# amazon-science/gan-control

Measured on AMD Instinct MI355X. Metric: images/sec G+D step FFHQ-1024, higher is better.
Workload: dtype bf16x3; 1 GPU; FFHQ 1024x1024 full G+D train step (D step, G step, lazy R1 every 16 and path-length every 4, Adam, EMA), 4 images/GPU, fp32 storage, conv arithmetic bf16x3; global_batch=4, parallelism=dp1

## Files before the change

### gan-control_amd/csrc/bias_act.hip

```cpp
#include "common.h"

namespace {

__device__ __forceinline__ float lrelu_gain(float v, float slope, float gain) {
    return (v > 0.f ? v : v * slope) * gain;
}

template <bool VEC, bool NOISE>
__global__ __launch_bounds__(256) void bias_act_plane_kernel(
    const float* __restrict__ x, const float* __restrict__ bias, const float* __restrict__ noise,
    const float* __restrict__ noise_w, float* __restrict__ y, int channels, int64_t inner, float slope, float gain) {
    const int plane = blockIdx.y;
    const int c = plane % channels, b = plane / channels;
    const float bv = bias ? bias[c] : 0.f;
    const float nw = NOISE ? noise_w[0] : 0.f;
    const float* xp = x + (size_t)plane * inner;
    float* yp = y + (size_t)plane * inner;
    const float* np = NOISE ? noise + (size_t)b * inner : nullptr;
    if (VEC) {
        const int64_t n4 = inner >> 2;
        for (int64_t i = (int64_t)blockIdx.x * 256 + threadIdx.x; i < n4; i += (int64_t)gridDim.x * 256) {
            const gc::f32x4_t xv = gc::stream_load4(xp + 4 * i);
            float4 v = make_float4(xv.x, xv.y, xv.z, xv.w);
            if (NOISE) {
// ... 487 lines not shown
    int chunks, rpc;
    plane_dot_pitched_plan(rows, &chunks, &rpc);
    return chunks;
}

extern "C" int gc_plane_dot_pitched_f32(const float* a, const float* b, float* partial, int planes, int rows, int width, int a_pitch, int b_pitch,
                                        gc_stream_t stream) {
    if (!a || !b || !partial) return gc::fail(GC_ERR_BAD_ARG, "gc_plane_dot_pitched_f32: null pointer");
    if (planes <= 0 || rows <= 0 || width <= 0 || a_pitch < width || b_pitch < width) return gc::fail(GC_ERR_BAD_ARG, "gc_plane_dot_pitched_f32: bad extents");
    int chunks, rpc;
    plane_dot_pitched_plan(rows, &chunks, &rpc);
    if ((int64_t)planes * chunks > INT32_MAX) return gc::fail(GC_ERR_UNSUPPORTED, "gc_plane_dot_pitched_f32: more than 2^31 blocks");
    hipLaunchKernelGGL(plane_dot_pitched_kernel, dim3((unsigned)planes * (unsigned)chunks), dim3(256), 0, (hipStream_t)stream,
                       a, b, partial, rows, width, a_pitch, b_pitch, chunks, rpc);
    return gc::check_launch("gc_plane_dot_pitched_f32");
}

extern "C" int gc_rows_sum_div_f32(const float* partial, const float* den, float* out, int rows, int chunks, gc_stream_t stream) {
    if (!partial || !out) return gc::fail(GC_ERR_BAD_ARG, "gc_rows_sum_div_f32: null pointer");
    if (rows <= 0 || chunks <= 0) return gc::fail(GC_ERR_BAD_ARG, "gc_rows_sum_div_f32: bad extents");
    hipLaunchKernelGGL(rows_sum_div_kernel, dim3((unsigned)((rows + 255) / 256)), dim3(256), 0, (hipStream_t)stream, partial, den, out, rows, chunks);
    return gc::check_launch("gc_rows_sum_div_f32");
}

extern "C" int gc_plane_dot_f32(const float* a, const float* b, float* partial, int planes, int64_t inner, gc_stream_t stream) {
    if (!a || !b || !partial) return gc::fail(GC_ERR_BAD_ARG, "gc_plane_dot_f32: null pointer");
    if (planes <= 0 || inner <= 0) return gc::fail(GC_ERR_BAD_ARG, "gc_plane_dot_f32: bad extents");
    int chunks; int64_t len;
    channel_sum_plan(inner, &chunks, &len);
    if ((int64_t)planes * chunks > INT32_MAX) return gc::fail(GC_ERR_UNSUPPORTED, "gc_plane_dot_f32: more than 2^31 blocks");
    hipLaunchKernelGGL(plane_dot_kernel, dim3((unsigned)chunks * (unsigned)planes), dim3(256), 0, (hipStream_t)stream, a, b, partial, inner, chunks, len);
    return gc::check_launch("gc_plane_dot_f32");
}
```

### gan-control_amd/gan_control_amd/_lib.py

```python
import ctypes
import os

import torch

_HERE = os.path.dirname(os.path.abspath(__file__))
_DEFAULT = os.path.normpath(os.path.join(_HERE, '..', 'csrc', 'libgancontrol_hip.so'))

ABI_VERSION = 2
MODE_IDS = {'f32': 0, 'bf16x3': 1, 'bf16': 2}

_i32, _i64, _f32, _vp, _sz = ctypes.c_int32, ctypes.c_int64, ctypes.c_float, ctypes.c_void_p, ctypes.c_size_t


class ConvDesc(ctypes.Structure):
    _fields_ = [(n, _i32) for n in ('batch', 'in_ch', 'out_ch', 'in_h', 'in_w', 'out_h', 'out_w',
                                    'kh', 'kw', 'up', 'down', 'pad_y', 'pad_x', 'in_pitch', 'out_pitch')]


class ConvEpilogue(ctypes.Structure):
    _fields_ = [('bias', _vp), ('noise', _vp), ('noise_w', _vp), ('slope', _f32), ('gain', _f32), ('activate', _i32), ('residual', _vp)]


class GlinGroup(ctypes.Structure):
    _fields_ = [('x', _vp), ('w', _vp), ('bias', _vp), ('y', _vp), ('n', _i32), ('k', _i32), ('x_stride', _i64), ('alpha', _f32), ('beta', _f32)]


class WLayoutGroup(ctypes.Structure):
    _fields_ = [('src', _vp), ('dst', _vp), ('taps', _i32), ('k', _i32), ('n', _i32), ('flip_taps', _i32), ('src_stride', _i64 * 3), ('dst_stride', _i64 * 3), ('scale', _f32)]


class WPackGroup(ctypes.Structure):
    _fields_ = [('desc', ConvDesc), ('w', _vp), ('packed', _vp), ('packed_bytes', _sz)]


class WsqGroup(ctypes.Structure):
    _fields_ = [('w', _vp), ('g', _vp), ('out', _vp), ('rows', _i32), ('taps', _i32)]


STRUCTS = (ConvDesc, ConvEpilogue, WLayoutGroup, WPackGroup, GlinGroup, WsqGroup)

SIGNATURES = {
    'gc_abi_version': (_i32, []),
    'gc_last_error': (ctypes.c_char_p, []),
    'gc_struct_sizes': (_i32, [ctypes.POINTER(_sz), _i32]),
    'gc_source_hash': (ctypes.c_char_p, []),
    'gc_upfirdn2d_f32': (_i32, [_vp, _vp, _vp] + [_i32] * 14 + [_vp]),
    'gc_upfirdn2d_act_f32': (_i32, [_vp, _vp, _vp] + [_i32] * 11 + [_vp, _vp, _vp, _f32, _f32, _vp]),
    'gc_bias_act_f32': (_i32, [_vp, _vp, _vp, _vp, _vp, _i32, _i32, _i64, _f32, _f32, _vp]),
    'gc_bias_act_bwd_f32': (_i32, [_vp, _vp, _vp, _i64, _f32, _f32, _vp]),
    'gc_bias_act_bwd_noise_f32': (_i32, [_vp, _vp, _vp, _vp, _vp, _i32, _i32, _i64, _f32, _f32, _vp]),
    'gc_bias_act_bwd_chunks': (_i32, [_i64]),
    'gc_bias_act_bwd_reduce_f32': (_i32, [_vp, _vp, _vp, _vp, _vp, _vp, _i32, _i32, _i64, _f32, _f32, _vp]),
    'gc_bias_act_bwd_reduce_self_f32': (_i32, [_vp, _vp, _vp, _vp, _vp, _vp, _vp, _vp, _vp, _i32, _i32, _i64, _f32, _f32, _vp]),
    'gc_bias_act_bwd_reduce_adjoint_f32': (_i32, [_vp] * 13 + [_i32, _i32, _i64, _f32, _f32, _vp]),
    'gc_plane_dot_f32': (_i32, [_vp, _vp, _vp, _i32, _i64, _vp]),
    'gc_rows_sum_div_f32': (_i32, [_vp, _vp, _vp, _i32, _i32, _vp]),
    'gc_conv2d_bn_relu_f32': (_i32, [_vp, _vp, _vp, _vp, _vp] + [_i32] * 13 + [_vp]),
    'gc_pool2d_f32': (_i32, [_vp, _vp] + [_i32] * 10 + [_vp]),
    'gc_global_avgpool_f32': (_i32, [_vp, _vp, _i32, _i32, _vp]),
    'gc_resize_bilinear_f32': (_i32, [_vp, _vp, _i32, _i32, _i32, _i32, _i32, _f32, _f32, _vp]),
    'gc_channel_sum_workspace': (_sz, [_i32, _i32, _i64]),
    'gc_channel_sum_f32': (_i32, [_vp, _vp, _i32, _i32, _i64, _vp, _sz, _vp]),
    'gc_conv2d_f32': (_i32, [ctypes.POINTER(ConvDesc), _vp, _vp, _vp, _vp, _vp, _vp]),
    'gc_conv2d_fused_f32': (_i32, [ctypes.POINTER(ConvDesc), _vp, _vp, _vp, _vp, ctypes.POINTER(ConvEpilogue), _vp, _vp]),
    'gc_conv2d_f32_workspace': (_sz, [ctypes.POINTER(ConvDesc)]),
    'gc_small_gemm_ok': (_i32, [_i32, _i32, _i32, _i64, _i64]),
    'gc_small_gemm_f32': (_i32, [_vp, _i64, _i64, _vp, _i64, _i64, _vp, _f32, _f32, _vp, _i32, _i32, _i32, _vp]),
    'gc_conv2d_fused_f32_ws': (_i32, [ctypes.POINTER(ConvDesc), _vp, _vp, _vp, _vp, ctypes.POINTER(ConvEpilogue), _vp, _vp, _sz, _vp]),
    'gc_conv2d_fused_bf16x3_f32': (_i32, [ctypes.POINTER(ConvDesc), _vp, _vp, _vp, _vp, ctypes.POINTER(ConvEpilogue), _vp, _vp, _sz, _vp]),
    'gc_conv2d_bf16x3_workspace': (_sz, [ctypes.POINTER(ConvDesc)]),
    'gc_conv2d_bf16x3_packed_bytes': (_sz, [ctypes.POINTER(ConvDesc)]),
    'gc_conv2d_bf16x3_splitk_bytes': (_sz, [ctypes.POINTER(ConvDesc)]),
    'gc_conv2d_pack_weights_bf16x3': (_i32, [ctypes.POINTER(ConvDesc), _vp, _vp, _sz, _vp]),
    'gc_conv2d_fused_bf16x3_packed_f32': (_i32, [ctypes.POINTER(ConvDesc), _vp, _vp, _vp, _sz, _vp, _vp, ctypes.POINTER(ConvEpilogue), _vp, _vp, _sz, _vp]),
    'gc_conv2d_fused_bf16_packed_f32': (_i32, [ctypes.POINTER(ConvDesc), _vp, _vp, _vp, _sz, _vp, _vp, ctypes.POINTER(ConvEpilogue), _vp, _vp, _sz, _vp]),
    'gc_conv2d_wgrad_bf16_f32': (_i32, [ctypes.POINTER(ConvDesc), _vp, _vp, _vp, _vp, _vp, _vp, _sz, _vp]),
    'gc_conv2d_variant_name': (_i32, [ctypes.POINTER(ConvDesc), _i32, ctypes.c_char_p, _i32]),
    'gc_conv2d_wgrad_variant_name': (_i32, [ctypes.POINTER(ConvDesc), _i32, _i32, ctypes.c_char_p, _i32]),
    'gc_conv2d_out_pitch': (_i32, [ctypes.POINTER(ConvDesc), _i32]),
    'gc_conv2d_in_pitch_ok': (_i32, [ctypes.POINTER(ConvDesc), _i32, _i32]),
    'gc_upfirdn2d_variant_name': (_i32, [_i32] * 7 + [ctypes.c_char_p, _i32]),
    'gc_upfirdn2d_actbwd_tiles': (_i32, [_i32, _i32]),
    'gc_upfirdn2d_actbwd_f32': (_i32, [_vp] * 7 + [_i32] * 12 + [_f32, _f32, _vp]),
    'gc_upfirdn2d_mask_f32': (_i32, [_vp, _vp, _vp] + [_i32] * 12 + [_vp, _f32, _f32, _vp]),
    'gc_upfirdn2d_pitched_f32': (_i32, [_vp, _vp, _vp] + [_i32] * 14 + [_vp, _vp, _vp, _f32, _f32, _vp]),
    'gc_plane_dot_pitched_chunks': (_i32, [_i32]),
    'gc_plane_dot_pitched_f32': (_i32, [_vp, _vp, _vp, _i32, _i32, _i32, _i32, _i32, _vp]),
    'gc_conv2d_bf16x3_f32': (_i32, [ctypes.POINTER(ConvDesc), _vp, _vp, _vp, _vp, _vp, _vp, _sz, _vp]),
    'gc_conv2d_wgrad_workspace': (_sz, [ctypes.POINTER(ConvDesc)]),
# ... 142 lines not shown
```

### gan-control_amd/gan_control_amd/models/op/modulated_conv.py

```python
import math
import os

import torch
from torch.autograd import Function

from . import _backend
from ._backend import ConvGeom
from .conv2d_gradfix import _adjoint_geom, _adjoint_weight
from .weight_layout import kernel_layout
from .upfirdn2d import upfirdn2d, _dense_or_pitched


_WGRAD_SAMPLES = int(os.environ.get('GANCONTROL_WGRAD_SAMPLES', '1'))
_SAMPLES_MIN_RATIO = float(os.environ.get('GANCONTROL_WGRAD_SAMPLES_RATIO', '2'))


def _samples_route(x, gy, g, want_si, want_so, derived=False):
    if not _WGRAD_SAMPLES or torch.is_grad_enabled() or not (want_si or want_so) or (derived and _WGRAD_SAMPLES < 2):
        return False
    be = _backend.get()
    if not hasattr(be, 'conv2d_wgrad_samples_bytes'):
        return False
    saved = 2.0 * ((x.numel() if want_si else 0) + (gy.numel() if want_so else 0))
    extra = 3.0 * x.shape[0] * g.kh * g.kw * x.shape[1] * gy.shape[1]
    if saved < _SAMPLES_MIN_RATIO * extra:
        return False
    if g.up == 1:
        return be.conv2d_wgrad_samples_bytes(_dense_or_pitched(x), gy, g) > 0
    return be.conv2d_wgrad_samples_bytes(_dense_or_pitched(gy), x, _swapped_geom(g, x)) > 0


def _weight_and_scale_grads(x, gy, w_t, si, so, g, want_si, want_so):
    be = _backend.get()
    cs = lambda t: None if t is None else t.contiguous()
    if g.up == 1:
        gw, dws = be.conv2d_wgrad_samples(_dense_or_pitched(x), _dense_or_pitched(gy), cs(si), cs(so), g)
        gsi, gso = be.wgrad_samples_contract(dws, w_t.contiguous(), cs(si), cs(so), want_si, want_so)
        return gw, gsi, gso
    dw_adj, dws = be.conv2d_wgrad_samples(_dense_or_pitched(gy), _dense_or_pitched(x), cs(so), cs(si), _swapped_geom(g, x))
# ... 46 lines not shown
        ws = ctx.saved_tensors
        be = _backend.get()
        if torch.is_grad_enabled() or getattr(be, 'weight_sq_bwd', None) is None or not all(w.is_contiguous() for w in ws):
            return tuple((2.0 * g)[:, :, None, None] * w if ctx.needs_input_grad[i] else None for i, (g, w) in enumerate(zip(gs, ws)))
        idx = [i for i in range(len(ws)) if ctx.needs_input_grad[i]]
        outs = be.weight_sq_bwd([ws[i] for i in idx], [gs[i].contiguous() for i in idx]) if idx else []
        res = [None] * len(ws)
        for i, o in zip(idx, outs):
            res[i] = o
        return tuple(res)


def weight_sq_all(weights):
    return list(_backend.call(_WeightSqAll, *[w.view(w.shape[-4:]) for w in weights]))


def demod_coefficients(weight, s, scale, eps=1e-8):
    wsq = _backend.call(_WeightSq, weight.view(weight.shape[1:]))
    from .linear import equal_linear
    return torch.rsqrt(equal_linear(s.pow(2), wsq, _eps_vector(s, wsq.shape[0], eps), scale * scale, 1.0))


_EPS_VECTORS = {}


def _eps_vector(like, n, eps):
    key = (like.device, like.dtype, n, eps)
    t = _EPS_VECTORS.get(key)
    if t is None:
        t = _EPS_VECTORS[key] = torch.full((n,), eps, device=like.device, dtype=like.dtype)
    return t


class _SafeDiv(Function):

    @staticmethod
    def forward(ctx, num, den):
        out = _backend.get().rows_sum_div(num.contiguous().unsqueeze(-1), den.contiguous())
        ctx.save_for_backward(den, out)
        ctx.set_materialize_grads(False)
        return out

    @staticmethod
    def backward(ctx, g):
        if g is None:
            return None, None
        den, out = ctx.saved_tensors
        gq = _backend.call(_SafeDiv, g, den)
        return (gq if ctx.needs_input_grad[0] else None), (-(gq * out) if ctx.needs_input_grad[1] else None)


class _SumDiv(Function):

    @staticmethod
    def forward(ctx, partial, den):
        out = _backend.get().rows_sum_div(partial.contiguous(), den.contiguous())
        ctx.save_for_backward(den, out)
        ctx.chunks = partial.shape[-1]
        ctx.set_materialize_grads(False)
        return out

    @staticmethod
    def backward(ctx, g):
        if g is None:
            return None, None
        den, out = ctx.saved_tensors
        gq = _backend.call(_SafeDiv, g, den)
        return (gq.unsqueeze(-1).expand(*gq.shape, ctx.chunks) if ctx.needs_input_grad[0] else None), (-(gq * out) if ctx.needs_input_grad[1] else None)


class _PlaneDot(Function):

    @staticmethod
    def forward(ctx, a, b, den=None):
        out = _backend.get().plane_dot(_dense_or_pitched(a), _dense_or_pitched(b), den)
        ctx.has_den = den is not None
        ctx.save_for_backward(a, b, den if den is not None else a.new_empty(0), out if den is not None else a.new_empty(0))
        ctx.set_materialize_grads(False)
        return out

    @staticmethod
    def backward(ctx, g):
        if g is None:
            return None, None, None
        a, b, den, out = ctx.saved_tensors
        gq = _backend.call(_SafeDiv, g, den) if ctx.has_den else g
        g4 = gq[:, :, None, None]
        return (g4 * b if ctx.needs_input_grad[0] else None), (g4 * a if ctx.needs_input_grad[1] else None), \
            (-(gq * out) if ctx.has_den and ctx.needs_input_grad[2] else None)


class _ModConv(Function):

    @staticmethod
    def forward(ctx, x, w_t, si, so, geom, bias=None, residual=None, fork=False, derived=False):
        ctx.derived = derived
        ep = None
        if bias is not None or residual is not None:
            ep = (bias, None, None, 1.0, 1.0, False, None if residual is None else residual.contiguous())
        y = _backend.get().conv2d(_dense_or_pitched(x), w_t.contiguous(), None if si is None else si.contiguous(),
                                  None if so is None else so.contiguous(), geom, epilogue=ep)
        ctx.geom, ctx.in_hw = geom, (x.shape[2], x.shape[3])
        ctx.has_si, ctx.has_so, ctx.has_bias, ctx.has_res = si is not None, so is not None, bias is not None, residual is not None
        ctx.set_materialize_grads(False)
        empty = x.new_empty(0)
        keep_res = residual if (residual is not None and so is not None) else empty
        keep_bias = bias if (bias is not None and so is not None) else empty
        ctx.save_for_backward(x, w_t, si if si is not None else empty, so if so is not None else empty, y, keep_res, keep_bias)
        return (y, x.view_as(x)) if fork else y

    @staticmethod
    def backward(ctx, gy, gfork=None):
        x, w_t, si, so, y, res, bias = ctx.saved_tensors
        si = si if ctx.has_si else None
        so = so if ctx.has_so else None
        g = ctx.geom
        need = ctx.needs_input_grad
        gx = gw = gsi = gso = gb = gres = None
        if gy is None:
            return (gfork if need[0] else None), None, None, None, None, None, None, None, None
        need_si = ctx.has_si and need[2]
        need_so = ctx.has_so and need[3]
        fused = need[1] and _backend.want_param_grads() and _samples_route(x, gy, g, need_si, need_so, ctx.derived)
        if need[0] or (need_si and not fused):
            gx = _backend.call(_ModConv, gy, _adjoint_weight(w_t), so, si, _adjoint_geom(g, *ctx.in_hw), None, gfork if need[0] else None, False, True)
        if fused:
            gw, gsi, gso = _weight_and_scale_grads(x, gy, w_t, si, so, g, need_si, need_so)
            need_si = need_so = False
        elif need[1] and _backend.want_param_grads():
            gw = _mod_weight_grad(x, gy, si, so, g)
        if need_si:
            conv_part = gx if (gfork is None or not need[0]) else gx - gfork
            gsi = _backend.call(_PlaneDot, x, conv_part, si)
        if need_so:
            conv_part = y
            if ctx.has_res:
                conv_part = conv_part - res
            if ctx.has_bias:
                conv_part = conv_part - bias.reshape(1, -1, 1, 1)
            gso = _backend.call(_PlaneDot, gy, conv_part, so)
        if ctx.has_bias and need[5] and _backend.want_param_grads():
            from .fused_act import _channel_sum
            gb = _channel_sum(gy)
        if ctx.has_res and need[6]:
            gres = gy
        return (gx if need[0] else None), gw, gsi, gso, None, gb, gres, None, None


class _ModConvAct(Function):

    @staticmethod
    def forward(ctx, x, w_t, si, so, bias, noise, noise_w, geom, slope, gain):
        out = _backend.get().conv2d(x.contiguous(), w_t.contiguous(), None if si is None else si.contiguous(),
                                    None if so is None else so.contiguous(), geom,
                                    epilogue=(bias, None if noise is None else noise.contiguous(), noise_w, slope, gain, True))
        ctx.geom, ctx.in_hw, ctx.cfg = geom, (x.shape[2], x.shape[3]), (slope, gain)
        ctx.has = (si is not None, so is not None, bias is not None, noise is not None)
        empty = x.new_empty(0)
        ctx.save_for_backward(x, w_t, *[t if t is not None else empty for t in (si, so, bias, noise, noise_w)], out)
        ctx.set_materialize_grads(False)
        return out

    @staticmethod
    def backward(ctx, gy):
        from .fused_act import _BiasActGrad, _BiasActGradReduce
        from . import noise_grad
        x, w_t, si, so, bias, noise, noise_w, out = ctx.saved_tensors
        has_si, has_so, has_bias, has_noise = ctx.has
        si, so, bias = (si if has_si else None), (so if has_so else None), (bias if has_bias else None)
        noise, noise_w = (noise, noise_w) if has_noise else (None, None)
        g, (slope, gain) = ctx.geom, ctx.cfg
        need = ctx.needs_input_grad
        gx = gw = gsi = gso = gb = gnw = gn = None
        if gy is None or not any(need[:7]):
            return (None,) * 10
        want_so = has_so and need[3]
        want_n = has_noise and need[5]
        if not _backend.want_param_grads():
            need = list(need)
            need[1] = need[4] = need[6] = False
        if (has_bias and need[4]) or (has_noise and need[6]) or want_so:
            g_pre, psum, pdot, pself = _backend.call(_BiasActGradReduce, gy, out, noise, slope, gain, bias, noise_w, want_so)
            if has_bias and need[4]:
                gb = psum.sum((0, 2))
            if has_noise and need[6]:
                gnw = pdot.sum().reshape(noise_w.shape)
            if want_so:
                gso = _backend.call(_SumDiv, pself, so)
            if want_n:
                gn = noise_grad.pixel_sums_once(g_pre, noise_w)
        elif want_n and not torch.is_grad_enabled():
            g_pre, gn = noise_grad.masked(gy, out, noise_w, slope, gain)
        else:
            g_pre = _backend.call(_BiasActGrad, gy, out, slope, gain)
            if want_n:
                gn = noise_grad.pixel_sums_once(g_pre, noise_w)
        if gn is not None:
            gn = gn.reshape(noise.shape)
        need_si = has_si and need[2]
        fused = need[1] and _samples_route(x, g_pre, g, need_si, False)
        if need[0] or (need_si and not fused):
            gx = _backend.call(_ModConv, g_pre, _adjoint_weight(w_t), so, si, _adjoint_geom(g, *ctx.in_hw), None, None, False, True)
        if fused:
            gw, gsi, _ = _weight_and_scale_grads(x, g_pre, w_t, si, so, g, True, False)
        elif need[1]:
            gw = _mod_weight_grad(x, g_pre, si, so, g)
        if need_si and not fused:
            gsi = _backend.call(_PlaneDot, x, gx, si)
        return (gx if need[0] else None), gw, gsi, gso, gb, gn, gnw, None, None, None


def _swapped_geom(g, x):
    return ConvGeom(g.kh, g.kw, 1, g.up, g.kh - 1 - g.pad_y, g.kw - 1 - g.pad_x, x.shape[2], x.shape[3])


def _mod_weight_grad(x, gy, si, so, g):
    if g.up == 1:
        return _backend.call(_ModWGrad, x, gy, si, so, g)
    return _adjoint_weight(_backend.call(_ModWGrad, gy, x, so, si, _swapped_geom(g, x)))


class _ModWGrad(Function):

    @staticmethod
    def forward(ctx, x, gy, si, so, geom):
        ctx.geom, ctx.in_hw = geom, (x.shape[2], x.shape[3])
        ctx.has_si, ctx.has_so = si is not None, so is not None
        empty = x.new_empty(0)
        ctx.save_for_backward(x, gy, si if si is not None else empty, so if so is not None else empty)
        ctx.set_materialize_grads(False)
        return _backend.get().conv2d_wgrad(_dense_or_pitched(x), _dense_or_pitched(gy), None if si is None else si.contiguous(),
                                           None if so is None else so.contiguous(), geom)

    @staticmethod
    def backward(ctx, ggw):
        if ggw is None:
            return None, None, None, None, None
        x, gy, si, so = ctx.saved_tensors
        si = si if ctx.has_si else None
        so = so if ctx.has_so else None
        g = ctx.geom
        gx = ggy = gsi = gso = None
        need_si = ctx.has_si and ctx.needs_input_grad[2]
        need_so = ctx.has_so and ctx.needs_input_grad[3]
        if ctx.needs_input_grad[0] or need_si:
            gx = _backend.call(_ModConv, gy, _adjoint_weight(ggw), so, si, _adjoint_geom(g, *ctx.in_hw), None, None, False, True)
        if ctx.needs_input_grad[1] or need_so:
            ggy = _backend.call(_ModConv, x, ggw.contiguous(), si, so, g, None, None, False, True)
        if need_si:
            gsi = _backend.call(_PlaneDot, x, gx, si)
        if need_so:
            gso = _backend.call(_PlaneDot, gy, ggy, so)
        return (gx if ctx.needs_input_grad[0] else None), (ggy if ctx.needs_input_grad[1] else None), gsi, gso, None


def modulated_conv2d(x, weight, s, demodulate=True, upsample=False, blur_kernel=None, blur_pad=None, padding=None, apply_blur=True,
                     bias=None, residual=None, fork=False, demod=None):
    _, oc, ic, k, _ = weight.shape
    scale = 1.0 / math.sqrt(ic * k * k)
    d = (demod if demod is not None else demod_coefficients(weight, s, scale)) if demodulate else None
    if upsample:
        if bias is not None or residual is not None or fork:
            raise NotImplementedError('modulated_conv2d: bias / residual / fork are built for the plain branch only')
        w_t = kernel_layout(weight.view(oc, ic, k, k), scale, flip=True)
        oh, ow = (x.shape[2] - 1) * 2 + k, (x.shape[3] - 1) * 2 + k
        y = _backend.call(_ModConv, x, w_t, s, d, ConvGeom(k, k, 2, 1, k - 1, k - 1, oh, ow))
        return upfirdn2d(y, blur_kernel, pad=blur_pad) if apply_blur else y
    pad = k // 2 if padding is None else padding
    w_t = kernel_layout(weight.view(oc, ic, k, k), scale)
    oh, ow = x.shape[2] + 2 * pad - k + 1, x.shape[3] + 2 * pad - k + 1
    if bias is None and residual is None and not fork:
        return _backend.call(_ModConv, x, w_t, s, d, ConvGeom(k, k, 1, 1, pad, pad, oh, ow))
    return _backend.call(_ModConv, x, w_t, s, d, ConvGeom(k, k, 1, 1, pad, pad, oh, ow), None if bias is None else bias.reshape(-1).contiguous(), residual, bool(fork))


def modulated_conv2d_act(x, weight, s, bias, noise, noise_weight, demodulate=True, padding=None, negative_slope=0.2, act_scale=2 ** 0.5, demod=None):
    _, oc, ic, k, _ = weight.shape
    scale = 1.0 / math.sqrt(ic * k * k)
# ... 9 lines not shown
```

### include/gancontrol_hip.h

```cpp
#ifndef GANCONTROL_HIP_H
#define GANCONTROL_HIP_H

#include <stddef.h>
#include <stdint.h>

#ifdef __cplusplus
extern "C" {
#endif

#define GC_ABI_VERSION 2

#define GC_OK 0
#define GC_ERR_BAD_ARG (-1)
#define GC_ERR_UNSUPPORTED (-2)
#define GC_ERR_HIP (-3)
#define GC_ERR_WORKSPACE (-4)

typedef void* gc_stream_t;

int gc_abi_version(void);
const char* gc_last_error(void);
#define GC_STRUCT_COUNT 6
int gc_struct_sizes(size_t* sizes, int n);
const char* gc_source_hash(void);
// ... 23 lines not shown
int gc_upfirdn2d_actbwd_f32(const float* gy, const float* y_ref, const float* noise, const float* taps, float* gx, float* psum, float* pdot,
                            int batch, int channels, int in_h, int in_w, int out_h, int out_w, int out_pitch, int kh, int kw,
                            int pad_x0, int pad_y0, int flip_taps, float slope, float gain, gc_stream_t stream);

int gc_bias_act_f32(const float* x, const float* bias, const float* noise, const float* noise_w,
                    float* y, int batch, int channels, int64_t inner,
                    float slope, float gain, gc_stream_t stream);

int gc_bias_act_bwd_f32(const float* dy, const float* y_ref, float* dx, int64_t count,
                        float slope, float gain, gc_stream_t stream);

int gc_bias_act_bwd_noise_f32(const float* dy, const float* y_ref, const float* noise_w, float* dx, float* dnoise,
                              int batch, int channels, int64_t inner, float slope, float gain, gc_stream_t stream);

int gc_bias_act_bwd_chunks(int64_t inner);
int gc_bias_act_bwd_reduce_f32(const float* dy, const float* y_ref, const float* noise, float* dx,
                               float* psum, float* pdot, int batch, int channels, int64_t inner,
                               float slope, float gain, gc_stream_t stream);

int gc_bias_act_bwd_reduce_self_f32(const float* dy, const float* y_ref, const float* noise, const float* bias, const float* noise_w,
                                    float* dx, float* psum, float* pdot, float* pself, int batch, int channels, int64_t inner,
                                    float slope, float gain, gc_stream_t stream);

int gc_bias_act_bwd_reduce_adjoint_f32(const float* ggx, const float* cs, const float* cd, const float* cw, const float* y_ref, const float* dx,
                                       const float* noise, const float* bias, const float* noise_w, float* g_dy, float* g_yref, float* pgb, float* pgn,
                                       int batch, int channels, int64_t inner, float slope, float gain, gc_stream_t stream);

int gc_plane_dot_f32(const float* a, const float* b, float* partial, int planes, int64_t inner, gc_stream_t stream);

int gc_plane_dot_pitched_chunks(int rows);
int gc_plane_dot_pitched_f32(const float* a, const float* b, float* partial, int planes, int rows, int width, int a_pitch, int b_pitch, gc_stream_t stream);

int gc_rows_sum_div_f32(const float* partial, const float* den, float* out, int rows, int chunks, gc_stream_t stream);

size_t gc_channel_sum_workspace(int batch, int channels, int64_t inner);
int gc_channel_sum_f32(const float* x, float* out, int batch, int channels, int64_t inner,
                       void* workspace, size_t workspace_bytes, gc_stream_t stream);

typedef struct gc_conv_desc {
    int32_t batch;
    int32_t in_ch, out_ch;
    int32_t in_h, in_w;
    int32_t out_h, out_w;
    int32_t kh, kw;
    int32_t up, down;
    int32_t pad_y, pad_x;
    int32_t in_pitch;
    int32_t out_pitch;
} gc_conv_desc;

int gc_small_gemm_ok(int M, int K, int N, int64_t sb0, int64_t sb1);
int gc_small_gemm_f32(const float* a, int64_t sa0, int64_t sa1, const float* b, int64_t sb0, int64_t sb1,
                      const float* bias, float beta, float alpha, float* out, int M, int K, int N, gc_stream_t stream);

int gc_conv2d_out_pitch(const gc_conv_desc* d, int mode);

int gc_conv2d_in_pitch_ok(const gc_conv_desc* d, int mode, int wgrad);

int gc_conv2d_f32(const gc_conv_desc* d, const float* x, const float* w,
                  const float* in_scale, const float* out_scale, float* y, gc_stream_t stream);

typedef struct gc_conv_epilogue {
    const float* bias;
    const float* noise;
    const float* noise_w;
    float slope, gain;
// ... 187 lines not shown
```

Before: 81.67 images/sec.

## Fuse per-plane scale, dot-with-subtract and quotient-gradient tails in modulated conv backward

Adds HIP kernels that fuse several elementwise and reduction tails in the modulated-conv double-backward path. One kernel does a per-plane scaled axpy for two outputs in one pass. Another computes a plane dot product of a against (b - c - bias) without materialising the difference. A third finishes the row-sum division and the negated quotient gradient in one launch. The goal is fewer kernel launches and fewer temporary full-size tensors in the R1 and path-length regularisation backward passes. The cost is extra code paths with eager fallbacks, gated by an environment flag that is on by default.

```diff
diff --git a/gan-control_amd/csrc/bias_act.hip b/gan-control_amd/csrc/bias_act.hip
--- a/gan-control_amd/csrc/bias_act.hip
+++ b/gan-control_amd/csrc/bias_act.hip
@@ -543,3 +543,230 @@
     hipLaunchKernelGGL(plane_dot_kernel, dim3((unsigned)chunks * (unsigned)planes), dim3(256), 0, (hipStream_t)stream, a, b, partial, inner, chunks, len);
     return gc::check_launch("gc_plane_dot_f32");
 }
+
+__global__ __launch_bounds__(256) void plane_dot_bwd_axpy_kernel(const float* __restrict__ coef, const float* __restrict__ x, const float* __restrict__ g, const float* acc,
+                                                         float* t, float* __restrict__ u, int64_t inner, int chunks, int64_t chunk_len) {
+    const int plane = blockIdx.x / chunks, j = blockIdx.x - plane * chunks;
+    const size_t base = (size_t)plane * inner;
+    const int64_t lo = (int64_t)j * chunk_len, hi = min(inner, lo + chunk_len);
+    const float c = coef[plane];
+    typedef float f4u __attribute__((ext_vector_type(4), aligned(4)));
+    const int64_t n4 = (hi - lo) >> 2;
+    for (int64_t v = threadIdx.x; v < n4; v += 256) {
+        const size_t i = base + lo + 4 * v;
+        if (t) {
+            const f4u x4 = gc::stream_load4u(x + i);
+            f4u r = {__fmul_rn(c, x4.x), __fmul_rn(c, x4.y), __fmul_rn(c, x4.z), __fmul_rn(c, x4.w)};
+            if (acc) {
+                const f4u a4 = *reinterpret_cast<const f4u*>(acc + i);
+                r = f4u{__fadd_rn(a4.x, r.x), __fadd_rn(a4.y, r.y), __fadd_rn(a4.z, r.z), __fadd_rn(a4.w, r.w)};
+            }
+            gc::stream_store4u(t + i, r.x, r.y, r.z, r.w);
+        }
+        if (u) {
+            const f4u g4 = gc::stream_load4u(g + i);
+            gc::stream_store4u(u + i, __fmul_rn(c, g4.x), __fmul_rn(c, g4.y), __fmul_rn(c, g4.z), __fmul_rn(c, g4.w));
+        }
+    }
+    for (int64_t k = lo + 4 * n4 + threadIdx.x; k < hi; k += 256) {
+        const size_t i = base + k;
+        if (t) {
+            const float p = __fmul_rn(c, x[i]);
+            t[i] = acc ? __fadd_rn(acc[i], p) : p;
+        }
+        if (u) u[i] = __fmul_rn(c, g[i]);
+    }
+}
+
+__global__ __launch_bounds__(256) void plane_dot_bwd_axpy_pitched_kernel(const float* __restrict__ coef, const float* __restrict__ x, const float* __restrict__ g, const float* acc,
+                                                                 float* t, float* __restrict__ u, int rows, int width, int x_pitch, int g_pitch, int acc_pitch,
+                                                                 int t_pitch, int u_pitch, int chunks, int rpc) {
+    const int plane = blockIdx.x / chunks, j = blockIdx.x - plane * chunks;
+    const int r0 = j * rpc, r1 = min(rows, r0 + rpc);
+    const float c = coef[plane];
+    typedef float f4u __attribute__((ext_vector_type(4), aligned(4)));
+    const int lane = threadIdx.x & 63, wave = threadIdx.x >> 6;
+    const int w4 = width >> 2;
+    const size_t prow = (size_t)plane * rows;
+    for (int r = r0 + wave; r < r1; r += 4) {
+        const float* xr = t ? x + (prow + r) * x_pitch : nullptr;
+        const float* ar = acc ? acc + (prow + r) * acc_pitch : nullptr;
+        float* tr = t ? t + (prow + r) * t_pitch : nullptr;
+        const float* gr = u ? g + (prow + r) * g_pitch : nullptr;
+        float* ur = u ? u + (prow + r) * u_pitch : nullptr;
+        for (int v = lane; v < w4; v += 64) {
+            if (t) {
+                const f4u x4 = *reinterpret_cast<const f4u*>(xr + 4 * v);
+                f4u q = {__fmul_rn(c, x4.x), __fmul_rn(c, x4.y), __fmul_rn(c, x4.z), __fmul_rn(c, x4.w)};
+                if (acc) {
+                    const f4u a4 = *reinterpret_cast<const f4u*>(ar + 4 * v);
+                    q = f4u{__fadd_rn(a4.x, q.x), __fadd_rn(a4.y, q.y), __fadd_rn(a4.z, q.z), __fadd_rn(a4.w, q.w)};
+                }
+                *reinterpret_cast<f4u*>(tr + 4 * v) = q;
+            }
+            if (u) {
+                const f4u g4 = *reinterpret_cast<const f4u*>(gr + 4 * v);
+                *reinterpret_cast<f4u*>(ur + 4 * v) = f4u{__fmul_rn(c, g4.x), __fmul_rn(c, g4.y), __fmul_rn(c, g4.z), __fmul_rn(c, g4.w)};
+            }
+        }
+        for (int k = 4 * w4 + lane; k < width; k += 64) {
+            if (t) {
+                const float p = __fmul_rn(c, xr[k]);
+                tr[k] = acc ? __fadd_rn(ar[k], p) : p;
+            }
+            if (u) ur[k] = __fmul_rn(c, gr[k]);
+        }
+    }
+}
+
+__global__ __launch_bounds__(256) void plane_dot_sub_kernel(const float* __restrict__ a, const float* __restrict__ b, const float* __restrict__ c,
+                                                            const float* __restrict__ bias, float* __restrict__ partial, int channels,
+                                                            int64_t inner, int chunks, int64_t chunk_len) {
+    __shared__ float lds[4];
+    const int plane = blockIdx.x / chunks, j = blockIdx.x - plane * chunks;
+    const size_t base = (size_t)plane * inner;
+    const int64_t lo = (int64_t)j * chunk_len, hi = min(inner, lo + chunk_len);
+    const bool has_bias = bias != nullptr;
+    const float bv = has_bias ? bias[plane % channels] : 0.f;
+    float acc = 0.f;
+    typedef float f4u __attribute__((ext_vector_type(4), aligned(4)));
+    const int64_t n4 = (hi - lo) >> 2;
+    for (int64_t v = threadIdx.x; v < n4; v += 256) {
+        const int64_t i = lo + 4 * v;
+        const f4u a4 = gc::stream_load4u(a + base + i);
+        f4u b4 = gc::stream_load4u(b + base + i);
+        if (c) {
+            const f4u c4 = gc::stream_load4u(c + base + i);
+            b4 = f4u{__fsub_rn(b4.x, c4.x), __fsub_rn(b4.y, c4.y), __fsub_rn(b4.z, c4.z), __fsub_rn(b4.w, c4.w)};
+        }
+        if (has_bias) b4 = f4u{__fsub_rn(b4.x, bv), __fsub_rn(b4.y, bv), __fsub_rn(b4.z, bv), __fsub_rn(b4.w, bv)};
+        acc = fmaf(a4.x, b4.x, acc); acc = fmaf(a4.y, b4.y, acc); acc = fmaf(a4.z, b4.z, acc); acc = fmaf(a4.w, b4.w, acc);
+    }
+    for (int64_t i = lo + 4 * n4 + threadIdx.x; i < hi; i += 256) {
+        float d = b[base + i];
+        if (c) d = __fsub_rn(d, c[base + i]);
+        if (has_bias) d = __fsub_rn(d, bv);
+        acc = fmaf(a[base + i], d, acc);
+    }
+    const float r = block_sum(acc, lds);
+    if (threadIdx.x == 0) partial[(size_t)plane * chunks + j] = r;
+}
+
+__global__ __launch_bounds__(256) void plane_dot_sub_pitched_kernel(const float* __restrict__ a, const float* __restrict__ b, const float* __restrict__ c,
+                                                                    const float* __restrict__ bias, float* __restrict__ partial, int channels, int rows, int width,
+                                                                    int a_pitch, int b_pitch, int c_pitch, int chunks, int rpc) {
+    __shared__ float lds[4];
+    const int plane = blockIdx.x / chunks, j = blockIdx.x - plane * chunks;
+    const float* ap = a + (size_t)plane * rows * a_pitch;
+    const float* bp = b + (size_t)plane * rows * b_pitch;
+    const float* cp = c ? c + (size_t)plane * rows * c_pitch : nullptr;
+    const bool has_bias = bias != nullptr;
+    const float bv = has_bias ? bias[plane % channels] : 0.f;
+    const int r0 = j * rpc, r1 = min(rows, r0 + rpc);
+    typedef float f4u __attribute__((ext_vector_type(4), aligned(4)));
+    const int lane = threadIdx.x & 63, wave = threadIdx.x >> 6;
+    const int w4 = width >> 2;
+    float acc0 = 0.f, acc1 = 0.f;
+    auto second = [&](const float* br, const float* cr, int v) {
+        f4u b4 = *reinterpret_cast<const f4u*>(br + 4 * v);
+        if (cr) {
+            const f4u c4 = *reinterpret_cast<const f4u*>(cr + 4 * v);
+            b4 = f4u{__fsub_rn(b4.x, c4.x), __fsub_rn(b4.y, c4.y), __fsub_rn(b4.z, c4.z), __fsub_rn(b4.w, c4.w)};
+        }
+        if (has_bias) b4 = f4u{__fsub_rn(b4.x, bv), __fsub_rn(b4.y, bv), __fsub_rn(b4.z, bv), __fsub_rn(b4.w, bv)};
+        return b4;
+    };
+    for (int r = r0 + wave; r < r1; r += 4) {
+        const float* ar = ap + (size_t)r * a_pitch;
+        const float* br = bp + (size_t)r * b_pitch;
+        const float* cr = cp ? cp + (size_t)r * c_pitch : nullptr;
+        int v = lane;
+        for (; v + 64 < w4; v += 128) {
+            const f4u a0 = *reinterpret_cast<const f4u*>(ar + 4 * v), b0 = second(br, cr, v);
+            const f4u a1 = *reinterpret_cast<const f4u*>(ar + 4 * (v + 64)), b1 = second(br, cr, v + 64);
+            acc0 = fmaf(a0.x, b0.x, acc0); acc0 = fmaf(a0.y, b0.y, acc0); acc0 = fmaf(a0.z, b0.z, acc0); acc0 = fmaf(a0.w, b0.w, acc0);
+            acc1 = fmaf(a1.x, b1.x, acc1); acc1 = fmaf(a1.y, b1.y, acc1); acc1 = fmaf(a1.z, b1.z, acc1); acc1 = fmaf(a1.w, b1.w, acc1);
+        }
+        for (; v < w4; v += 64) {
+            const f4u a0 = *reinterpret_cast<const f4u*>(ar + 4 * v), b0 = second(br, cr, v);
+            acc0 = fmaf(a0.x, b0.x, acc0); acc0 = fmaf(a0.y, b0.y, acc0); acc0 = fmaf(a0.z, b0.z, acc0); acc0 = fmaf(a0.w, b0.w, acc0);
+        }
+        for (int k = 4 * w4 + lane; k < width; k += 64) {
+            float d = br[k];
+            if (cr) d = __fsub_rn(d, cr[k]);
+            if (has_bias) d = __fsub_rn(d, bv);
+            acc1 = fmaf(ar[k], d, acc1);
+        }
+    }
+    const float s = block_sum(acc0 + acc1, lds);
+    if (threadIdx.x == 0) partial[(size_t)plane * chunks + j] = s;
+}
+
+__global__ __launch_bounds__(256) void rows_sum_div_pair_kernel(const float* __restrict__ partial, const float* __restrict__ den, const float* __restrict__ saved,
+                                                                float* __restrict__ out, float* __restrict__ neg, int rows, int chunks) {
+    const int r = blockIdx.x * 256 + threadIdx.x;
+    if (r >= rows) return;
+    float acc = 0.f;
+    for (int j = 0; j < chunks; ++j) acc += partial[(size_t)r * chunks + j];
+    if (den) { const float d = den[r]; acc = acc / (d == 0.f ? 1.f : d); }
+    out[r] = acc;
+    neg[r] = -__fmul_rn(acc, saved[r]);
+}
+
+extern "C" int gc_plane_axpy_f32(const float* coef, const float* x, const float* g, const float* acc, float* t, float* u, int planes, int64_t inner,
+                                 gc_stream_t stream) {
+    if (!coef || (!t && !u)) return gc::fail(GC_ERR_BAD_ARG, "gc_plane_axpy_f32: null pointer");
+    if ((t && !x) || (u && !g) || (acc && !t)) return gc::fail(GC_ERR_BAD_ARG, "gc_plane_axpy_f32: t needs x, u needs g, acc needs t");
+    if (planes <= 0 || inner <= 0) return gc::fail(GC_ERR_BAD_ARG, "gc_plane_axpy_f32: bad extents");
+    int chunks; int64_t len;
+    channel_sum_plan(inner, &chunks, &len);
+    if ((int64_t)planes * chunks > INT32_MAX) return gc::fail(GC_ERR_UNSUPPORTED, "gc_plane_axpy_f32: more than 2^31 blocks");
+    hipLaunchKernelGGL(plane_dot_bwd_axpy_kernel, dim3((unsigned)chunks * (unsigned)planes), dim3(256), 0, (hipStream_t)stream, coef, x, g, acc, t, u, inner, chunks, len);
+    return gc::check_launch("gc_plane_axpy_f32");
+}
+
+extern "C" int gc_plane_axpy_pitched_f32(const float* coef, const float* x, const float* g, const float* acc, float* t, float* u, int planes, int rows, int width,
+                                         int x_pitch, int g_pitch, int acc_pitch, int t_pitch, int u_pitch, gc_stream_t stream) {
+    if (!coef || (!t && !u)) return gc::fail(GC_ERR_BAD_ARG, "gc_plane_axpy_pitched_f32: null pointer");
+    if ((t && !x) || (u && !g) || (acc && !t)) return gc::fail(GC_ERR_BAD_ARG, "gc_plane_axpy_pitched_f32: t needs x, u needs g, acc needs t");
+    if (planes <= 0 || rows <= 0 || width <= 0) return gc::fail(GC_ERR_BAD_ARG, "gc_plane_axpy_pitched_f32: bad extents");
+    if ((t && (x_pitch < width || t_pitch < width)) || (acc && acc_pitch < width) || (u && (g_pitch < width || u_pitch < width)))
+        return gc::fail(GC_ERR_BAD_ARG, "gc_plane_axpy_pitched_f32: a pitch below the width");
+    int chunks, rpc;
+    plane_dot_pitched_plan(rows, &chunks, &rpc);
+    if ((int64_t)planes * chunks > INT32_MAX) return gc::fail(GC_ERR_UNSUPPORTED, "gc_plane_axpy_pitched_f32: more than 2^31 blocks");
+    hipLaunchKernelGGL(plane_dot_bwd_axpy_pitched_kernel, dim3((unsigned)planes * (unsigned)chunks), dim3(256), 0, (hipStream_t)stream, coef, x, g, acc, t, u, rows, width,
+                       x_pitch, g_pitch, acc_pitch, t_pitch, u_pitch, chunks, rpc);
+    return gc::check_launch("gc_plane_axpy_pitched_f32");
+}
+
+extern "C" int gc_plane_dot_sub_f32(const float* a, const float* b, const float* c, const float* bias, float* partial, int planes, int channels, int64_t inner,
+                                    gc_stream_t stream) {
+    if (!a || !b || !partial) return gc::fail(GC_ERR_BAD_ARG, "gc_plane_dot_sub_f32: null pointer");
+    if (planes <= 0 || inner <= 0 || channels <= 0 || planes % channels) return gc::fail(GC_ERR_BAD_ARG, "gc_plane_dot_sub_f32: bad extents");
+    int chunks; int64_t len;
+    channel_sum_plan(inner, &chunks, &len);
+    if ((int64_t)planes * chunks > INT32_MAX) return gc::fail(GC_ERR_UNSUPPORTED, "gc_plane_dot_sub_f32: more than 2^31 blocks");
+    hipLaunchKernelGGL(plane_dot_sub_kernel, dim3((unsigned)chunks * (unsigned)planes), dim3(256), 0, (hipStream_t)stream, a, b, c, bias, partial, channels, inner, chunks, len);
+    return gc::check_launch("gc_plane_dot_sub_f32");
+}
+
+extern "C" int gc_plane_dot_sub_pitched_f32(const float* a, const float* b, const float* c, const float* bias, float* partial, int planes, int channels, int rows,
+                                            int width, int a_pitch, int b_pitch, int c_pitch, gc_stream_t stream) {
+    if (!a || !b || !partial) return gc::fail(GC_ERR_BAD_ARG, "gc_plane_dot_sub_pitched_f32: null pointer");
+    if (planes <= 0 || rows <= 0 || width <= 0 || channels <= 0 || planes % channels || a_pitch < width || b_pitch < width || (c && c_pitch < width))
+        return gc::fail(GC_ERR_BAD_ARG, "gc_plane_dot_sub_pitched_f32: bad extents");
+    int chunks, rpc;
+    plane_dot_pitched_plan(rows, &chunks, &rpc);
+    if ((int64_t)planes * chunks > INT32_MAX) return gc::fail(GC_ERR_UNSUPPORTED, "gc_plane_dot_sub_pitched_f32: more than 2^31 blocks");
+    hipLaunchKernelGGL(plane_dot_sub_pitched_kernel, dim3((unsigned)planes * (unsigned)chunks), dim3(256), 0, (hipStream_t)stream, a, b, c, bias, partial, channels,
+                       rows, width, a_pitch, b_pitch, c_pitch, chunks, rpc);
+    return gc::check_launch("gc_plane_dot_sub_pitched_f32");
+}
+
+extern "C" int gc_rows_sum_div_pair_f32(const float* partial, const float* den, const float* saved, float* out, float* neg, int rows, int chunks, gc_stream_t stream) {
+    if (!partial || !saved || !out || !neg) return gc::fail(GC_ERR_BAD_ARG, "gc_rows_sum_div_pair_f32: null pointer");
+    if (rows <= 0 || chunks <= 0) return gc::fail(GC_ERR_BAD_ARG, "gc_rows_sum_div_pair_f32: bad extents");
+    hipLaunchKernelGGL(rows_sum_div_pair_kernel, dim3((unsigned)((rows + 255) / 256)), dim3(256), 0, (hipStream_t)stream, partial, den, saved, out, neg, rows, chunks);
+    return gc::check_launch("gc_rows_sum_div_pair_f32");
+}
diff --git a/gan-control_amd/gan_control_amd/_lib.py b/gan-control_amd/gan_control_amd/_lib.py
--- a/gan-control_amd/gan_control_amd/_lib.py
+++ b/gan-control_amd/gan_control_amd/_lib.py
@@ -55,6 +55,11 @@
     'gc_bias_act_bwd_reduce_adjoint_f32': (_i32, [_vp] * 13 + [_i32, _i32, _i64, _f32, _f32, _vp]),
     'gc_plane_dot_f32': (_i32, [_vp, _vp, _vp, _i32, _i64, _vp]),
     'gc_rows_sum_div_f32': (_i32, [_vp, _vp, _vp, _i32, _i32, _vp]),
+    'gc_rows_sum_div_pair_f32': (_i32, [_vp, _vp, _vp, _vp, _vp, _i32, _i32, _vp]),
+    'gc_plane_axpy_f32': (_i32, [_vp] * 6 + [_i32, _i64, _vp]),
+    'gc_plane_axpy_pitched_f32': (_i32, [_vp] * 6 + [_i32] * 8 + [_vp]),
+    'gc_plane_dot_sub_f32': (_i32, [_vp] * 5 + [_i32, _i32, _i64, _vp]),
+    'gc_plane_dot_sub_pitched_f32': (_i32, [_vp] * 5 + [_i32] * 7 + [_vp]),
     'gc_conv2d_bn_relu_f32': (_i32, [_vp, _vp, _vp, _vp, _vp] + [_i32] * 13 + [_vp]),
     'gc_pool2d_f32': (_i32, [_vp, _vp] + [_i32] * 10 + [_vp]),
     'gc_global_avgpool_f32': (_i32, [_vp, _vp, _i32, _i32, _vp]),
diff --git a/gan-control_amd/gan_control_amd/models/op/modulated_conv.py b/gan-control_amd/gan_control_amd/models/op/modulated_conv.py
--- a/gan-control_amd/gan_control_amd/models/op/modulated_conv.py
+++ b/gan-control_amd/gan_control_amd/models/op/modulated_conv.py
@@ -5,6 +5,7 @@
 from torch.autograd import Function
 
 from . import _backend
+from . import plane_ops
 from ._backend import ConvGeom
 from .conv2d_gradfix import _adjoint_geom, _adjoint_weight
 from .weight_layout import kernel_layout
@@ -117,6 +118,13 @@
     return t
 
 
+def _quotient_grads(g, den, out, want_den):
+    if want_den and plane_ops.FUSE and plane_ops.native(g, den, out):
+        return plane_ops.rows_sum_div_pair(g.contiguous().unsqueeze(-1), den, out)
+    gq = _backend.call(_SafeDiv, g, den)
+    return gq, (-(gq * out) if want_den else None)
+
+
 class _SafeDiv(Function):
 
     @staticmethod
@@ -131,8 +139,8 @@
         if g is None:
             return None, None
         den, out = ctx.saved_tensors
-        gq = _backend.call(_SafeDiv, g, den)
-        return (gq if ctx.needs_input_grad[0] else None), (-(gq * out) if ctx.needs_input_grad[1] else None)
+        gq, gden = _quotient_grads(g, den, out, ctx.needs_input_grad[1])
+        return (gq if ctx.needs_input_grad[0] else None), gden
 
 
 class _SumDiv(Function):
@@ -150,29 +158,50 @@
         if g is None:
             return None, None
         den, out = ctx.saved_tensors
-        gq = _backend.call(_SafeDiv, g, den)
-        return (gq.unsqueeze(-1).expand(*gq.shape, ctx.chunks) if ctx.needs_input_grad[0] else None), (-(gq * out) if ctx.needs_input_grad[1] else None)
+        gq, gden = _quotient_grads(g, den, out, ctx.needs_input_grad[1])
+        return (gq.unsqueeze(-1).expand(*gq.shape, ctx.chunks) if ctx.needs_input_grad[0] else None), gden
 
 
 class _PlaneDot(Function):
 
     @staticmethod
-    def forward(ctx, a, b, den=None):
-        out = _backend.get().plane_dot(_dense_or_pitched(a), _dense_or_pitched(b), den)
-        ctx.has_den = den is not None
-        ctx.save_for_backward(a, b, den if den is not None else a.new_empty(0), out if den is not None else a.new_empty(0))
+    def forward(ctx, a, b, den=None, minus=None, bias=None):
+        if minus is None and bias is None:
+            out = _backend.get().plane_dot(_dense_or_pitched(a), _dense_or_pitched(b), den)
+        else:
+            out = plane_ops.plane_dot_sub(_dense_or_pitched(a), _dense_or_pitched(b), None if minus is None else _dense_or_pitched(minus), bias, den)
+        ctx.has_den, ctx.has_minus, ctx.has_bias = den is not None, minus is not None, bias is not None
+        empty = a.new_empty(0)
+        ctx.save_for_backward(a, b, den if den is not None else empty, out if den is not None else empty,
+                              minus if minus is not None else empty, bias if bias is not None else empty)
         ctx.set_materialize_grads(False)
         return out
 
     @staticmethod
     def backward(ctx, g):
+        need = tuple(ctx.needs_input_grad) + (False,) * 5
+        n_in = len(ctx.needs_input_grad)
         if g is None:
-            return None, None, None
-        a, b, den, out = ctx.saved_tensors
-        gq = _backend.call(_SafeDiv, g, den) if ctx.has_den else g
+            return (None,) * n_in
+        a, b, den, out, minus, bias = ctx.saved_tensors
+        gq, gden = _quotient_grads(g, den, out, need[2]) if ctx.has_den else (g, None)
         g4 = gq[:, :, None, None]
-        return (g4 * b if ctx.needs_input_grad[0] else None), (g4 * a if ctx.needs_input_grad[1] else None), \
-            (-(gq * out) if ctx.has_den and ctx.needs_input_grad[2] else None)
+        ga = gb = gminus = gbias = None
+        if need[0]:
+            second = b
+            if ctx.has_minus:
+                second = second - minus
+            if ctx.has_bias:
+                second = second - bias.reshape(1, -1, 1, 1)
+            ga = g4 * second
+        want_minus, want_bias = ctx.has_minus and need[3], ctx.has_bias and need[4]
+        if need[1] or want_minus or want_bias:
+            gb = g4 * a
+        if want_minus or want_bias:
+            gneg = -gb
+            gminus = gneg if want_minus else None
+            gbias = gneg.sum((0, 2, 3)) if want_bias else None
+        return ((ga, gb if need[1] else None, gden, gminus, gbias))[:n_in]
 
 
 class _ModConv(Function):
@@ -207,29 +236,90 @@
         need_si = ctx.has_si and need[2]
         need_so = ctx.has_so and need[3]
         fused = need[1] and _backend.want_param_grads() and _samples_route(x, gy, g, need_si, need_so, ctx.derived)
-        if need[0] or (need_si and not fused):
-            gx = _backend.call(_ModConv, gy, _adjoint_weight(w_t), so, si, _adjoint_geom(g, *ctx.in_hw), None, gfork if need[0] else None, False, True)
+        residual = gfork if need[0] else None
+        if need_si and not fused and residual is None and _pair_node():
+            gx, gsi = _backend.call(_ModConvDot, gy, _adjoint_weight(w_t), so, si, si, x, _adjoint_geom(g, *ctx.in_hw))
+            need_si = False
+        elif need[0] or (need_si and not fused):
+            gx = _backend.call(_ModConv, gy, _adjoint_weight(w_t), so, si, _adjoint_geom(g, *ctx.in_hw), None, residual, False, True)
         if fused:
             gw, gsi, gso = _weight_and_scale_grads(x, gy, w_t, si, so, g, need_si, need_so)
             need_si = need_so = False
         elif need[1] and _backend.want_param_grads():
             gw = _mod_weight_grad(x, gy, si, so, g)
         if need_si:
-            conv_part = gx if (gfork is None or not need[0]) else gx - gfork
-            gsi = _backend.call(_PlaneDot, x, conv_part, si)
+            if residual is None:
+                gsi = _backend.call(_PlaneDot, x, gx, si)
+            elif plane_ops.FUSE:
+                gsi = _backend.call(_PlaneDot, x, gx, si, residual)
+            else:
+                gsi = _backend.call(_PlaneDot, x, gx - residual, si)
         if need_so:
-            conv_part = y
-            if ctx.has_res:
-                conv_part = conv_part - res
-            if ctx.has_bias:
-                conv_part = conv_part - bias.reshape(1, -1, 1, 1)
-            gso = _backend.call(_PlaneDot, gy, conv_part, so)
+            if plane_ops.FUSE and (ctx.has_res or ctx.has_bias):
+                gso = _backend.call(_PlaneDot, gy, y, so, res if ctx.has_res else None, bias if ctx.has_bias else None)
+            else:
+                conv_part = y
+                if ctx.has_res:
+                    conv_part = conv_part - res
+                if ctx.has_bias:
+                    conv_part = conv_part - bias.reshape(1, -1, 1, 1)
+                gso = _backend.call(_PlaneDot, gy, conv_part, so)
         if ctx.has_bias and need[5] and _backend.want_param_grads():
             from .fused_act import _channel_sum
             gb = _channel_sum(gy)
         if ctx.has_res and need[6]:
             gres = gy
         return (gx if need[0] else None), gw, gsi, gso, None, gb, gres, None, None
+
+
+def _pair_node():
+    return bool(plane_ops.FUSE) and torch.is_grad_enabled()
+
+
+class _ModConvDot(Function):
+
+    @staticmethod
+    def forward(ctx, x, w_t, si, so_dot, so, a, geom):
+        be = _backend.get()
+        y = be.conv2d(_dense_or_pitched(x), w_t.contiguous(), None if si is None else si.contiguous(), so.contiguous(), geom, epilogue=None)
+        dot = be.plane_dot(_dense_or_pitched(a), _dense_or_pitched(y), so_dot)
+        ctx.geom, ctx.in_hw, ctx.has_si = geom, (x.shape[2], x.shape[3]), si is not None
+        ctx.set_materialize_grads(False)
+        ctx.save_for_backward(x, w_t, si if si is not None else x.new_empty(0), so, y, a, dot)
+        return y, dot
+
+    @staticmethod
+    def backward(ctx, gy, gdot):
+        if gy is None and gdot is None:
+            return (None,) * 7
+        x, w_t, si, so, y, a, dot = ctx.saved_tensors
+        si = si if ctx.has_si else None
+        g = ctx.geom
+        need = ctx.needs_input_grad
+        ga = gso_dot = None
+        if gdot is not None:
+            c, gso_dot = _quotient_grads(gdot, so, dot, need[3])
+            if plane_ops.native(c, a, y, gy):
+                gy, ga = plane_ops.plane_axpy(c, _dense_or_pitched(a), gy, _dense_or_pitched(y) if need[5] else None)
+            else:
+                c4 = c[:, :, None, None]
+                ga = c4 * y if need[5] else None
+                gy = c4 * a if gy is None else gy + c4 * a
+        gx = gw = gsi = gso = None
+        need_si, need_so = ctx.has_si and need[2], need[4]
+        fused = need[1] and _backend.want_param_grads() and _samples_route(x, gy, g, need_si, need_so, True)
+        if need[0] or (need_si and not fused):
+            gx = _backend.call(_ModConv, gy, _adjoint_weight(w_t), so, si, _adjoint_geom(g, *ctx.in_hw), None, None, False, True)
+        if fused:
+            gw, gsi, gso = _weight_and_scale_grads(x, gy, w_t, si, so, g, need_si, need_so)
+            need_si = need_so = False
+        elif need[1] and _backend.want_param_grads():
+            gw = _mod_weight_grad(x, gy, si, so, g)
+        if need_si:
+            gsi = _backend.call(_PlaneDot, x, gx, si)
+        if need_so:
+            gso = _backend.call(_PlaneDot, gy, y, so)
+        return (gx if need[0] else None), gw, gsi, gso_dot, gso, ga, None
 
 
 class _ModConvAct(Function):
@@ -284,7 +374,10 @@
             gn = gn.reshape(noise.shape)
         need_si = has_si and need[2]
         fused = need[1] and _samples_route(x, g_pre, g, need_si, False)
-        if need[0] or (need_si and not fused):
+        if need_si and not fused and _pair_node():
+            gx, gsi = _backend.call(_ModConvDot, g_pre, _adjoint_weight(w_t), so, si, si, x, _adjoint_geom(g, *ctx.in_hw))
+            need_si = False
+        elif need[0] or (need_si and not fused):
             gx = _backend.call(_ModConv, g_pre, _adjoint_weight(w_t), so, si, _adjoint_geom(g, *ctx.in_hw), None, None, False, True)
         if fused:
             gw, gsi, _ = _weight_and_scale_grads(x, g_pre, w_t, si, so, g, True, False)
@@ -328,7 +421,10 @@
         gx = ggy = gsi = gso = None
         need_si = ctx.has_si and ctx.needs_input_grad[2]
         need_so = ctx.has_so and ctx.needs_input_grad[3]
-        if ctx.needs_input_grad[0] or need_si:
+        if need_si and _pair_node():
+            gx, gsi = _backend.call(_ModConvDot, gy, _adjoint_weight(ggw), so, si, si, x, _adjoint_geom(g, *ctx.in_hw))
+            need_si = False
+        elif ctx.needs_input_grad[0] or need_si:
             gx = _backend.call(_ModConv, gy, _adjoint_weight(ggw), so, si, _adjoint_geom(g, *ctx.in_hw), None, None, False, True)
         if ctx.needs_input_grad[1] or need_so:
             ggy = _backend.call(_ModConv, x, ggw.contiguous(), si, so, g, None, None, False, True)
diff --git a/gan-control_amd/gan_control_amd/models/op/plane_ops.py b/gan-control_amd/gan_control_amd/models/op/plane_ops.py
--- /dev/null
+++ b/gan-control_amd/gan_control_amd/models/op/plane_ops.py
@@ -0,0 +1,142 @@
+import os
+
+import torch
+
+from ... import _lib
+from . import _backend
+from ._backend import HipBackend
+
+FUSE = int(os.environ.get('GANCONTROL_FUSE_PLANE_TAIL', '1'))
+
+AXPY, AXPY_PITCHED = 'gc_plane_axpy_f32', 'gc_plane_axpy_pitched_f32'
+DOT_SUB, DOT_SUB_PITCHED = 'gc_plane_dot_sub_f32', 'gc_plane_dot_sub_pitched_f32'
+DIV_PAIR = 'gc_rows_sum_div_pair_f32'
+
+
+def native(*tensors):
+    if torch.is_grad_enabled() or getattr(_backend.get(), 'name', None) != 'hip':
+        return False
+    return all(t is None or (t.is_cuda and t.dtype == torch.float32) for t in tensors)
+
+
+def _pitch(t):
+    if t is None or t.dim() != 4 or t.is_contiguous():
+        return 0
+    b, c, h, w = t.shape
+    sb, sc, sh, sw = t.stride()
+    return sh if (sw == 1 and sh > w and sc == h * sh and sb == c * sc) else 0
+
+
+def _in_place(t):
+    return t if (t is None or t.is_contiguous() or _pitch(t)) else t.contiguous()
+
+
+def _planes(t):
+    b, c = t.shape[0], t.shape[1]
+    return b, c, t.numel() // max(b * c, 1)
+
+
+def plane_axpy(coef, x=None, acc=None, g=None, out=None):
+    if x is None and g is None:
+        raise ValueError('plane_axpy: one of x and g is required')
+    if acc is not None and x is None:
+        raise ValueError('plane_axpy: acc without x')
+    like = x if x is not None else g
+    if not native(coef, x, acc, g, out):
+        c4 = coef.reshape(tuple(coef.shape) + (1,) * (like.dim() - 2))
+        t = u = None
+        if x is not None:
+            t = c4 * x
+            if acc is not None:
+                t = acc + t
+            if out is not None:
+                t = out.copy_(t)
+        if g is not None:
+            u = c4 * g
+        return t, u
+    be = _backend.get()
+    coef, x, acc, g = coef.contiguous(), _in_place(x), _in_place(acc), _in_place(g)
+    like = x if x is not None else g
+    dev = _lib.require_cuda_f32(coef)
+    b, c, inner = _planes(like)
+    shape = tuple(like.shape)
+    for o in (x, acc, g, out):
+        if o is not None and (tuple(o.shape) != shape or o.device != dev):
+            raise ValueError('plane_axpy: operands of shapes %s on one device expected' % (shape,))
+    if tuple(coef.shape) != (b, c):
+        raise ValueError('plane_axpy: coef %s for planes %s' % (tuple(coef.shape), shape))
+    if out is not None and not (out.is_contiguous() or _pitch(out)):
+        raise ValueError('plane_axpy: out must be dense or row-pitched')
+    t = (out if out is not None else torch.empty(shape, dtype=torch.float32, device=dev)) if x is not None else None
+    u = torch.empty(shape, dtype=torch.float32, device=dev) if g is not None else None
+    if like.numel() == 0:
+        return t, u
+    pitches = [_pitch(o) for o in (x, g, acc, t, u)]
+    if any(pitches):
+        rows, width = shape[2], shape[3]
+        be._launch(dev, AXPY_PITCHED, _lib.ptr(coef), _lib.ptr(x), _lib.ptr(g), _lib.ptr(acc), _lib.ptr(t), _lib.ptr(u), b * c, rows, width,
+                   *[p or width for p in pitches], _lib.stream_of(like))
+    else:
+        be._launch(dev, AXPY, _lib.ptr(coef), _lib.ptr(x), _lib.ptr(g), _lib.ptr(acc), _lib.ptr(t), _lib.ptr(u), b * c, inner, _lib.stream_of(like))
+    return t, u
+
+
+def dot_sub_chunks(shape, pitched=False):
+    lib = _lib.load()
+    if pitched:
+        return lib.gc_plane_dot_pitched_chunks(shape[2])
+    b, c = shape[0], shape[1]
+    return lib.gc_bias_act_bwd_chunks(int(torch.Size(shape).numel()) // max(b * c, 1))
+
+
+def plane_dot_sub(a, b, minus=None, bias=None, den=None):
+    be = _backend.get()
+    if not native(a, b, minus, bias, den) or (not _pitch(a) and (_pitch(b) or _pitch(minus))):
+        from .upfirdn2d import _dense_or_pitched
+        d = b
+        if minus is not None:
+            d = d - minus
+        if bias is not None:
+            d = d - bias.reshape(1, -1, *([1] * (b.dim() - 2)))
+        return be.plane_dot(_dense_or_pitched(a), _dense_or_pitched(d), den)
+    a, b, minus = _in_place(a), _in_place(b), _in_place(minus)
+    bias = None if bias is None else bias.contiguous()
+    _lib.require_cuda_f32(bias, den)
+    dev = a.device
+    batch, ch, inner = _planes(a)
+    if tuple(b.shape) != tuple(a.shape) or (minus is not None and tuple(minus.shape) != tuple(a.shape)) or (bias is not None and bias.numel() != ch):
+        raise ValueError('plane_dot_sub: a %s, b %s, minus %s, bias %s' % tuple(None if o is None else tuple(o.shape) for o in (a, b, minus, bias)))
+    pa, pb, pm = _pitch(a), _pitch(b), _pitch(minus)
+    pitched = bool(pa or pb or pm)
+    chunks = dot_sub_chunks(a.shape, pitched)
+    partial = torch.empty((batch, ch, chunks), dtype=torch.float32, device=dev)
+    if a.numel():
+        if pitched:
+            rows, width = a.shape[2], a.shape[3]
+            be._launch(dev, DOT_SUB_PITCHED, _lib.ptr(a), _lib.ptr(b), _lib.ptr(minus), _lib.ptr(bias), _lib.ptr(partial), batch * ch, ch, rows, width,
+                       pa or width, pb or width, pm or width, _lib.stream_of(a))
+        else:
+            be._launch(dev, DOT_SUB, _lib.ptr(a), _lib.ptr(b), _lib.ptr(minus), _lib.ptr(bias), _lib.ptr(partial), batch * ch, ch, inner, _lib.stream_of(a))
+    if den is None and chunks == 1:
+        return partial.reshape(batch, ch)
+    return be.rows_sum_div(partial, None if den is None else den.contiguous())
+
+
+def rows_sum_div_pair(partial, den, saved):
+    if not native(partial, den, saved):
+        q = _backend.get().rows_sum_div(partial.contiguous(), None if den is None else den.contiguous())
+        return q, -(q * saved)
+    partial, saved = partial.contiguous(), saved.contiguous()
+    den = None if den is None else den.contiguous()
+    dev = _lib.require_cuda_f32(partial, den, saved)
+    lead = tuple(partial.shape[:-1])
+    rows, chunks = 1, int(partial.shape[-1])
+    for n in lead:
+        rows *= int(n)
+    if tuple(saved.shape) != lead or (den is not None and tuple(den.shape) != lead):
+        raise ValueError('rows_sum_div_pair: partial %s, den %s, saved %s' % (tuple(partial.shape), None if den is None else tuple(den.shape), tuple(saved.shape)))
+    q = torch.empty(lead, dtype=torch.float32, device=dev)
+    neg = torch.empty(lead, dtype=torch.float32, device=dev)
+    if rows:
+        _backend.get()._launch(dev, DIV_PAIR, _lib.ptr(partial), _lib.ptr(den), _lib.ptr(saved), _lib.ptr(q), _lib.ptr(neg), rows, chunks, _lib.stream_of(partial))
+    return q, neg
diff --git a/include/gancontrol_hip.h b/include/gancontrol_hip.h
--- a/include/gancontrol_hip.h
+++ b/include/gancontrol_hip.h
@@ -79,6 +79,17 @@
 int gc_plane_dot_pitched_f32(const float* a, const float* b, float* partial, int planes, int rows, int width, int a_pitch, int b_pitch, gc_stream_t stream);
 
 int gc_rows_sum_div_f32(const float* partial, const float* den, float* out, int rows, int chunks, gc_stream_t stream);
+
+int gc_rows_sum_div_pair_f32(const float* partial, const float* den, const float* saved, float* out, float* neg, int rows, int chunks, gc_stream_t stream);
+
+int gc_plane_axpy_f32(const float* coef, const float* x, const float* g, const float* acc, float* t, float* u, int planes, int64_t inner, gc_stream_t stream);
+int gc_plane_axpy_pitched_f32(const float* coef, const float* x, const float* g, const float* acc, float* t, float* u, int planes, int rows, int width,
+                              int x_pitch, int g_pitch, int acc_pitch, int t_pitch, int u_pitch, gc_stream_t stream);
+
+int gc_plane_dot_sub_f32(const float* a, const float* b, const float* c, const float* bias, float* partial, int planes, int channels, int64_t inner,
+                         gc_stream_t stream);
+int gc_plane_dot_sub_pitched_f32(const float* a, const float* b, const float* c, const float* bias, float* partial, int planes, int channels, int rows,
+                                 int width, int a_pitch, int b_pitch, int c_pitch, gc_stream_t stream);
 
 size_t gc_channel_sum_workspace(int batch, int channels, int64_t inner);
 int gc_channel_sum_f32(const float* x, float* out, int batch, int channels, int64_t inner,
```

Result: no change. 82.04 images/sec (median of 6 runs) (+0.5%).
